# Yusin2Chen/incomplete_multimodal_fusion

Hardware: AMD Instinct MI355X
Metric: pretrain_samples_per_sec (higher is better)
Workload: dtype bf16

## Files before the change

incomplete_multimodal_fusion_amd/csrc/mha_sh.hip:

```cpp
#include "mha_common.hpp"
#include "mmae_hip.h"

typedef short s16x4 __attribute__((ext_vector_type(4)));
typedef short s16x8 __attribute__((ext_vector_type(8)));
typedef float f32x16 __attribute__((ext_vector_type(16)));
typedef unsigned u32x4 __attribute__((ext_vector_type(4)));
typedef unsigned u32x2 __attribute__((ext_vector_type(2)));
typedef __bf16 bf16x2 __attribute__((ext_vector_type(2)));
#define LDS_AS __attribute__((address_space(3)))

#ifndef SH_SKEW
#define SH_SKEW 0
#endif
#ifndef SH_SLEEP_CLASS
#define SH_SLEEP_CLASS (-1)
#endif
#define SH_NS 4
#define SH_D 3
#define SH_MAXT 64
#define SH_MAXP 64
#define SH_LOG2E 1.4426950408889634f
#define SH_LN2 0.6931471805599453f
#define SH_THR 6.0f

__device__ __forceinline__ int sh_uni(int v) { return __builtin_amdgcn_readfirstlane(v); }
__device__ __forceinline__ int sh_f(int r) { return (((r >> 1) & 1) << 2) | (((r >> 2) & 1) << 1) | ((r >> 3) & 1); }
__device__ __forceinline__ float sh_exp2(float x) { return __builtin_amdgcn_exp2f(x); }
__device__ __forceinline__ f32x16 sh_mma(const bf16x8& a, const bf16x8& b, const f32x16& c) {
    return __builtin_amdgcn_mfma_f32_32x32x16_bf16(a, b, c, 0, 0, 0);
}
__device__ __forceinline__ float sh_swap_max(float v) {
    const unsigned w = __builtin_bit_cast(unsigned, v);
    auto b = __builtin_amdgcn_permlane32_swap(w, w, false, false);
    return fmaxf(__builtin_bit_cast(float, (unsigned)b[0]), __builtin_bit_cast(float, (unsigned)b[1]));
}
__device__ __forceinline__ float sh_swap_sum(float v) {
    const unsigned w = __builtin_bit_cast(unsigned, v);
    auto b = __builtin_amdgcn_permlane32_swap(w, w, false, false);
    return __builtin_bit_cast(float, (unsigned)b[0]) + __builtin_bit_cast(float, (unsigned)b[1]);
}
#define SH_W1(k) "s_waitcnt vmcnt(" #k ")\n\ts_branch .Lshw_end_%=\n\t"
#define SH_W4(a, b, c, d) SH_W1(a) SH_W1(b) SH_W1(c) SH_W1(d)
__device__ __forceinline__ void sh_wait_vm(int n) {
    int k = sh_uni(n < 0 ? 0 : (n > 31 ? 31 : n));
    asm volatile(
        "s_getpc_b64 vcc\n\t"
        "s_lshl_b32 %0, %0, 3\n\t"
        "s_add_u32 %0, %0, 20\n\t"
        "s_add_u32 vcc_lo, vcc_lo, %0\n\t"
        "s_addc_u32 vcc_hi, vcc_hi, 0\n\t"
        "s_setpc_b64 vcc\n\t"
        SH_W4(0, 1, 2, 3) SH_W4(4, 5, 6, 7) SH_W4(8, 9, 10, 11) SH_W4(12, 13, 14, 15)
        SH_W4(16, 17, 18, 19) SH_W4(20, 21, 22, 23) SH_W4(24, 25, 26, 27) SH_W4(28, 29, 30, 31)
        ".Lshw_end_%=:"
        : "+s"(k) : : "vcc", "scc", "memory");
}
__device__ __forceinline__ float sh_bf16_round(float x) { return (float)(bf16)x; }
__device__ __forceinline__ unsigned sh_pack2(float lo, float hi) {
    const unsigned a = __builtin_bit_cast(unsigned short, (bf16)lo), b = __builtin_bit_cast(unsigned short, (bf16)hi);
    return a | (b << 16);
}
__device__ __forceinline__ bf16x8 sh_ext(unsigned w0) { return __builtin_bit_cast(bf16x8, u32x4{w0, 0u, 0u, 0u}); }

struct ShSeg {
    int qlen, qst, klen, kst;
    __device__ __forceinline__ void load(const MhaDesc& p, int b, int lane) {
        const int i = b * p.nseg + (lane < p.nseg ? lane : 0);
        qlen = p.q_len[i]; qst = p.q_start[i]; klen = p.k_len[i]; kst = p.k_start[i];
    }
    __device__ __forceinline__ int ql(int s) const { return __builtin_amdgcn_readlane(qlen, sh_uni(s)); }
    __device__ __forceinline__ int qs(int s) const { return __builtin_amdgcn_readlane(qst, sh_uni(s)); }
    __device__ __forceinline__ int kl(int s) const { return __builtin_amdgcn_readlane(klen, sh_uni(s)); }
    __device__ __forceinline__ int ks(int s) const { return __builtin_amdgcn_readlane(kst, sh_uni(s)); }
};

__device__ __forceinline__ void sh_dma(const bf16* base, int n_rows, int row_bytes, int voff, int soff, bf16* lds_piece) {
    const unsigned long long a = reinterpret_cast<unsigned long long>(base);
    const unsigned lo = __builtin_amdgcn_readfirstlane((unsigned)a), hi = __builtin_amdgcn_readfirstlane((unsigned)(a >> 32));
    bf16* ub = reinterpret_cast<bf16*>(((unsigned long long)hi << 32) | lo);
    const __amdgpu_buffer_rsrc_t rs = __builtin_amdgcn_make_buffer_rsrc(ub, 0, sh_uni(n_rows * row_bytes), 0x00020000);
    __builtin_amdgcn_raw_ptr_buffer_load_lds(rs, (LDS_AS void*)lds_piece, 16, voff, sh_uni(soff), 0, 0);
}

__device__ __forceinline__ void sh_dma4(const float* base, int n, float* lds, int lane) {
    const unsigned long long a = reinterpret_cast<unsigned long long>(base);
    const unsigned lo = __builtin_amdgcn_readfirstlane((unsigned)a), hi = __builtin_amdgcn_readfirstlane((unsigned)(a >> 32));
    float* ub = reinterpret_cast<float*>(((unsigned long long)hi << 32) | lo);
    const __amdgpu_buffer_rsrc_t rs = __builtin_amdgcn_make_buffer_rsrc(ub, 0, sh_uni(n * 4), 0x00020000);
    int z = 0;
    asm volatile("" : "+s"(z));
    __builtin_amdgcn_raw_ptr_buffer_load_lds(rs, (LDS_AS void*)lds, 4, (lane + z) * 4, 0, 0, 0);
}

__device__ __forceinline__ u32x4 sh_rsrc_words(const void* base, int bytes) {
    const unsigned long long a = reinterpret_cast<unsigned long long>(base);
    return u32x4{(unsigned)__builtin_amdgcn_readfirstlane((unsigned)a), (unsigned)__builtin_amdgcn_readfirstlane((unsigned)(a >> 32)) & 0xffffu,
                 (unsigned)sh_uni(bytes), 0x00020000u};
}
__device__ __forceinline__ u32x4 sh_ld128_async(const void* base, int bytes, int voff) {
    u32x4 v;
    asm volatile("s_nop 4\n\tbuffer_load_dwordx4 %0, %1, %2, 0 offen" : "=&v"(v) : "v"(voff), "s"(sh_rsrc_words(base, bytes)) : "memory");
    return v;
}
__device__ __forceinline__ unsigned sh_ld32_async(const void* base, int bytes, int voff) {
    unsigned v;
    asm volatile("s_nop 4\n\tbuffer_load_dword %0, %1, %2, 0 offen" : "=&v"(v) : "v"(voff), "s"(sh_rsrc_words(base, bytes)) : "memory");
    return v;
}
__device__ __forceinline__ void sh_pin(u32x4& a, u32x4& b, unsigned& c) { asm volatile("" : "+v"(a), "+v"(b), "+v"(c)); }
template <int CTRL>
__device__ __forceinline__ float sh_add_dpp(float x) {
    return x + __builtin_bit_cast(float, __builtin_amdgcn_update_dpp(0, __builtin_bit_cast(int, x), CTRL, 0xf, 0xf, true));
}

__device__ __forceinline__ bf16x8 sh_tr(const bf16* img, int off0, int off1) {
    const s16x4 lo = __builtin_amdgcn_ds_read_tr16_b64_v4i16((LDS_AS s16x4*)(img + off0));
    const s16x4 hi = __builtin_amdgcn_ds_read_tr16_b64_v4i16((LDS_AS s16x4*)(img + off1));
    s16x8 x;
    x[0] = lo[0]; x[1] = lo[1]; x[2] = lo[2]; x[3] = lo[3]; x[4] = hi[0]; x[5] = hi[1]; x[6] = hi[2]; x[7] = hi[3];
    return __builtin_bit_cast(bf16x8, x);
}
__device__ __forceinline__ bf16x8 sh_ld8(const bf16* p) { return *reinterpret_cast<const bf16x8*>(p); }

struct ShAddr {
    int krow0, tr00;
    __device__ __forceinline__ void init(int lane) {
        const int r = lane & 31, hh = lane >> 5;
        krow0 = r * 64 + 8 * (hh ^ sh_f(r));
        const int g16 = lane >> 4, q = (lane & 15) >> 2, pp = lane & 3;
        const int row = 4 * (g16 >> 1) + q, ch = 2 * (g16 & 1) + (pp >> 1);
        tr00 = row * 64 + 8 * (ch ^ sh_f(row)) + 4 * (pp & 1);
    }
};

struct ShSlot {
    bf16x8 q[4];
    f32x16 o[2];
    float mref, lsum;
    unsigned ext;
    int row;
    int nq;
};

#ifndef MMAE_DIAG
#define MMAE_DIAG 1
#endif
#define SH_STAMP_WAVES (MMAE_DIAG ? 8192 : 1)
__device__ unsigned long long g_sh_stamps[SH_STAMP_WAVES][16];
__device__ __forceinline__ unsigned long long sh_now() {
    unsigned long long t;
    asm volatile("s_memtime %0\n\ts_waitcnt lgkmcnt(0)" : "=s"(t) :: "memory");
    return t;
}
extern "C" int mmae_debug_sh_stamps(unsigned long long* host32) {
    if (!host32 || !MMAE_DIAG) return MMAE_ERR_ARG;
    static unsigned long long* h = nullptr;
    if (!h) h = new unsigned long long[(size_t)SH_STAMP_WAVES * 16];
    if (hipMemcpyFromSymbol(h, HIP_SYMBOL(g_sh_stamps), sizeof(unsigned long long) * SH_STAMP_WAVES * 16) != hipSuccess) return MMAE_ERR_LAUNCH;
    for (int i = 0; i < 32; ++i) host32[i] = 0;
    for (size_t w = 0; w < SH_STAMP_WAVES; ++w)
        for (int i = 0; i < 16; ++i) host32[16 * ((w & 15) >= 8) + i] += h[w * 16 + i];
    void* dptr = nullptr;
    if (hipGetSymbolAddress(&dptr, HIP_SYMBOL(g_sh_stamps)) != hipSuccess) return MMAE_ERR_LAUNCH;
    if (hipMemset(dptr, 0, sizeof(unsigned long long) * SH_STAMP_WAVES * 16) != hipSuccess) return MMAE_ERR_LAUNCH;
    return MMAE_OK;
}
#define SH_T(i) do { if (ST) { __builtin_amdgcn_sched_barrier(0); const unsigned long long n__ = sh_now(); tt[i] += n__ - tl; tl = n__; __builtin_amdgcn_sched_barrier(0); } } while (0)

template <bool ST>
__device__ __forceinline__ void sh_attend(ShSlot& s, bool fresh, const bf16* Kst, const bf16* Vst, int stage_el, const ShAddr& ad,
                                          const unsigned (&kext)[2], int hh, unsigned long long (&tt)[16], unsigned long long& tl) {
    f32x16 sacc[2];
    const bf16x8 qe = sh_ext(s.ext);
    const int kbase = ad.krow0 + stage_el, vbase = ad.tr00 + stage_el;
    f32x16 z;
#pragma unroll
    for (int i = 0; i < 16; ++i) z[i] = 0.f;
#pragma unroll
    for (int kb = 0; kb < 2; ++kb) {
        bf16x8 kf[4];
#pragma unroll
        for (int ks = 0; ks < 4; ++ks) kf[ks] = sh_ld8(Kst + 2048 * kb + (kbase ^ (16 * ks)));
        sacc[kb] = sh_mma(sh_ext(kext[kb]), qe, z);
#pragma unroll
        for (int ks = 0; ks < 4; ++ks) sacc[kb] = sh_mma(kf[ks], s.q[ks], sacc[kb]);
        __builtin_amdgcn_sched_group_barrier(0x100, 4, 0);
        __builtin_amdgcn_sched_group_barrier(0x008, 5, 0);
    }
    if (ST) asm volatile("s_nop 15\n\ts_nop 15\n\ts_nop 15\n\ts_nop 15" ::: "memory");
    SH_T(4);
    float mx0 = fmaxf(sacc[0][0], sacc[0][1]), mx1 = fmaxf(sacc[1][0], sacc[1][1]);
#pragma unroll
    for (int i = 2; i < 16; i += 2) { mx0 = fmaxf(fmaxf(mx0, sacc[0][i]), sacc[0][i + 1]); mx1 = fmaxf(fmaxf(mx1, sacc[1][i]), sacc[1][i + 1]); }
    const float mx = sh_swap_max(fmaxf(mx0, mx1));
    const bool need = fresh | (mx > SH_THR);
    if (__builtin_amdgcn_ballot_w64(need) != 0) {
        const float want = s.mref + (fresh ? mx : fmaxf(mx, 0.f));
        const float mnew = sh_bf16_round(want);
        const float delta = mnew - s.mref;
        if (!fresh) {
            const float alpha = sh_exp2(-delta);
            s.lsum *= alpha;
#pragma unroll
            for (int d = 0; d < 2; ++d)
#pragma unroll
                for (int i = 0; i < 16; ++i) s.o[d][i] *= alpha;
        }
        s.mref = mnew;
        s.ext = hh == 0 ? sh_pack2(-mnew, 1.0f) : 0u;
#pragma unroll
        for (int kb = 0; kb < 2; ++kb)
#pragma unroll
            for (int i = 0; i < 16; ++i) sacc[kb][i] -= delta;
    }
    bf16x8 pb[2][2];
    const bf16x2 ones = {(bf16)1.0f, (bf16)1.0f};
#pragma unroll
    for (int kb = 0; kb < 2; ++kb) {
#pragma unroll
        for (int i = 0; i < 16; ++i) sacc[kb][i] = sh_exp2(sacc[kb][i]);
#pragma unroll
        for (int s2 = 0; s2 < 2; ++s2) {
#pragma unroll
            for (int j = 0; j < 8; ++j) pb[kb][s2][j] = (bf16)sacc[kb][8 * s2 + j];
            const u32x4 w = __builtin_bit_cast(u32x4, pb[kb][s2]);
#pragma unroll
            for (int j = 0; j < 4; ++j) s.lsum = __builtin_amdgcn_fdot2_f32_bf16(__builtin_bit_cast(bf16x2, (unsigned)w[j]), ones, s.lsum, false);
        }
    }
    SH_T(5);
#pragma unroll
    for (int kb = 0; kb < 2; ++kb) {
#pragma unroll
        for (int s2 = 0; s2 < 2; ++s2) {
            const bf16* vb = Vst + 64 * (32 * kb + 16 * s2);
            if (kb == 0 && s2 == 0 && fresh) {
#pragma unroll
                for (int d = 0; d < 2; ++d) s.o[d] = sh_mma(sh_tr(vb, vbase ^ (32 * d), vbase ^ (32 * d + 520)), pb[kb][s2], z);
            } else {
#pragma unroll
                for (int d = 0; d < 2; ++d) s.o[d] = sh_mma(sh_tr(vb, vbase ^ (32 * d), vbase ^ (32 * d + 520)), pb[kb][s2], s.o[d]);
            }
        }
        if (kb == 0) __builtin_amdgcn_sched_barrier(0);
    }
    if (ST) asm volatile("s_nop 15\n\ts_nop 15\n\ts_nop 15\n\ts_nop 15" ::: "memory");
    SH_T(6);
}

__device__ __forceinline__ void sh_finish(const ShSlot& s, const MhaDesc& p, int h, int r, int hh) {
    const float lq = sh_swap_sum(s.lsum);
    const float inv = lq > 0.f ? 1.f / lq : 0.f;
    const bool valid = r < s.nq;
    bf16* op = reinterpret_cast<bf16*>(p.o) + (long)s.row * p.o_stride + h * 64 + 8 * hh;
#pragma unroll
    for (int d = 0; d < 2; ++d)
#pragma unroll
        for (int i = 0; i < 4; i += 2) {
            unsigned a0 = sh_pack2(s.o[d][4 * i] * inv, s.o[d][4 * i + 1] * inv), a1 = sh_pack2(s.o[d][4 * i + 2] * inv, s.o[d][4 * i + 3] * inv);
            unsigned b0 = sh_pack2(s.o[d][4 * i + 4] * inv, s.o[d][4 * i + 5] * inv), b1 = sh_pack2(s.o[d][4 * i + 6] * inv, s.o[d][4 * i + 7] * inv);
            auto r0 = __builtin_amdgcn_permlane32_swap(a0, b0, false, false); a0 = r0[0]; b0 = r0[1];
            auto r1 = __builtin_amdgcn_permlane32_swap(a1, b1, false, false); a1 = r1[0]; b1 = r1[1];
            if (valid) *reinterpret_cast<u32x4*>(op + 32 * d + 8 * i) = u32x4{a0, a1, b0, b1};
        }
    if (valid && hh == 0) p.lse[(long)h * p.stat_stride + s.row] = lq > 0.f ? s.mref * SH_LN2 + __logf(lq) : 0.f;
}

__device__ __forceinline__ void sh_zero_rows(const MhaDesc& p, long row0, int n, int h, int tid) {
    for (int i = tid; i < n * 8; i += 1024) {
        const int rr = i >> 3, c = i & 7;
        *reinterpret_cast<u32x4*>(reinterpret_cast<bf16*>(p.o) + (row0 + rr) * p.o_stride + h * 64 + 8 * c) = u32x4{0u, 0u, 0u, 0u};
        if (c == 0) p.lse[(long)h * p.stat_stride + row0 + rr] = 0.f;
    }
}

// ... 779 lines not shown
        for (int s = 0; s < fus; ++s) {
            const int nb = (st.kl(s) + 31) >> 5;
            if (nb == 0) continue;
            const int room = (SB_W - NB % SB_W) % SB_W;
            if (room > 0 && nb > room && nb <= SB_W) {
                const int pad = min(room, FB - fus_used);
                if (pad > 0) { place(fus, fus_used, pad); fus_used += pad; }
            }
            place(s, 0, nb);
        }
        if (FB > fus_used) place(fus, fus_used, FB - fus_used);
        NB = min(NB, SB_MAXB);
        npass = (NB + SB_W - 1) / SB_W;
        if (wave == 0) { kb_row_s[lane] = kb_row; kb_info_s[lane] = kb_info; }
        unsigned firstp = 0, lastp = 0, seen = 0;
        for (int ps = 0; ps < npass; ++ps)
            for (int w = 0; w < SB_W; ++w) {
                const int kbi = SB_W * ps + w;
                if (kbi < NB) {
                    const int s = (__builtin_amdgcn_readlane(kb_info, kbi) >> 8) & 15;
                    if (!((seen >> s) & 1)) { seen |= 1u << s; firstp |= (unsigned)ps << (4 * s); }
                    lastp = (lastp & ~(15u << (4 * s))) | ((unsigned)ps << (4 * s));
                }
            }
        for (int ps = 0; ps < npass; ++ps) {
            int segmask = 0;
            for (int w = 0; w < SB_W; ++w) {
                const int kbi = SB_W * ps + w;
                if (kbi < NB) segmask |= 1 << ((__builtin_amdgcn_readlane(kb_info, kbi) >> 8) & 15);
            }
            const int first = nsteps;
            int tbase = 0;
            for (int sq = 0; sq < nseg; ++sq) {
                const int QL = st.ql(sq), nt = (QL + 63) >> 6;
                const int tb = tbase;
                tbase += nt;
                if (QL == 0) continue;
                int mode = 0;
                if (sq == fus) mode = 1;
                else if (st.kl(sq) > 0) mode = (segmask >> sq) & 1;
                else if (p.empty_mode == 0) mode = 2;
                if (!mode) continue;
                const int fp = sq == fus ? 0 : (int)((firstp >> (4 * sq)) & 15), lp = sq == fus ? npass - 1 : (int)((lastp >> (4 * sq)) & 15);
#pragma unroll
                for (int k = 0; k < 2; ++k) {
                    const int j = lane + 64 * k - nsteps;
                    if (j >= 0 && j < nt) {
                        st_row[k] = st.qs(sq) + 64 * j; st_tid[k] = tb + j;
                        st_info[k] = min(64, QL - 64 * j) | (sq << 8) | (mode << 12) | (ps << 16) | ((ps == fp ? 1 : 0) << 25) | ((ps == lp ? 1 : 0) << 26);
                    }
                }
                nsteps += nt;
            }
            if (nsteps == first) {
#pragma unroll
                for (int k = 0; k < 2; ++k)
                    if (lane + 64 * k == nsteps) { st_row[k] = 0; st_tid[k] = 0; st_info[k] = (3 << 12) | (ps << 16); }
                ++nsteps;
            }
#pragma unroll
            for (int k = 0; k < 2; ++k)
                if (lane + 64 * k == nsteps - 1) st_info[k] |= 1 << 24;
        }
        nsteps = min(nsteps, SB_MAXS);
    }
    __syncthreads();
    for (int hi = 0; hi < hpb; ++hi)
        for (int s = 0; s < nseg; ++s) {
            const int QL = st.ql(s);
            if (QL > 0 && (NB == 0 || (s < fus && st.kl(s) == 0))) {
                const long row0 = st.qs(s);
                for (int i = tid; i < QL * 8; i += SB_W * 64)
                    *reinterpret_cast<u32x4*>(reinterpret_cast<bf16*>(p.dq) + (row0 + (i >> 3)) * p.dq_stride + (h0 + hi) * 64 + 8 * (i & 7)) = u32x4{0u, 0u, 0u, 0u};
            }
        }
    if (NB == 0) return;
    auto s_row = [&](int i) { return i < 64 ? __builtin_amdgcn_readlane(st_row[0], i) : __builtin_amdgcn_readlane(st_row[1], i - 64); };
    auto s_info = [&](int i) { return i < 64 ? __builtin_amdgcn_readlane(st_info[0], i) : __builtin_amdgcn_readlane(st_info[1], i - 64); };
    auto s_tid = [&](int i) { return i < 64 ? __builtin_amdgcn_readlane(st_tid[0], i) : __builtin_amdgcn_readlane(st_tid[1], i - 64); };

    const bf16* qg = reinterpret_cast<const bf16*>(p.q);
    const bf16* dog = reinterpret_cast<const bf16*>(p.dout);
    const bf16* kg = reinterpret_cast<const bf16*>(p.k);
    const bf16* vg = reinterpret_cast<const bf16*>(p.v);
    const int qsb = (int)p.q_stride * 2, dosb = (int)p.do_stride * 2, ksb = (int)p.k_stride * 2, vsb = (int)p.v_stride * 2;
    auto dma_voff = [&](int row_bytes, int z) { const int pr = (lane >> 3) + z; return pr * row_bytes + 16 * ((lane & 7) ^ sh_f(pr)); };
    ShAddr ad; ad.init(lane);
    const float cq = p.scale * SH_LOG2E;
    const int G = hpb * nsteps;
    int vm = 0, myseq = 0, mark = 0;
    int lj = 0, li = 0, lh = 0, lstage = 0;
    auto issue_ring = [&]() {
        if (wave == 4 + (lj & 3)) {
            const long row0 = s_row(li); const int n = s_info(li) & 255, h = h0 + lh;
            const bf16* qb_ = qg + row0 * p.q_stride + h * 64;
            const bf16* ob_ = dog + row0 * p.do_stride + h * 64;
            int z = 0;
            asm volatile("" : "+s"(z));
            const int qv = dma_voff(qsb, z), ov = dma_voff(dosb, z);
#pragma unroll
            for (int pc = 0; pc < 8; ++pc) {
                sh_dma(qb_, n, qsb, qv ^ (16 * (pc & 1)), 8 * pc * qsb, &ringQ[lstage][pc * 512]);
                sh_dma(ob_, n, dosb, ov ^ (16 * (pc & 1)), 8 * pc * dosb, &ringO[lstage][pc * 512]);
            }
            if (!RC) {
                const float* lp = p.delta + ((long)p.H + h) * p.stat_stride + row0;
                const float* dp = p.delta + (2L * p.H + h) * p.stat_stride + row0;
                sh_dma4(lp, n, &ringL[lstage][0], lane);
                sh_dma4(dp, n, &ringL[lstage][64], lane);
            }
            vm += RC ? 16 : 18; myseq = vm;
        }
        ++lj;
        if (++lstage == SB_NS) lstage = 0;
        if (++li == nsteps) { li = 0; ++lh; }
    };
    u32x4 rc_o[2] = {{0u, 0u, 0u, 0u}, {0u, 0u, 0u, 0u}}, rc_d[2] = {{0u, 0u, 0u, 0u}, {0u, 0u, 0u, 0u}};
    unsigned rc_l = 0u;
    int rcseq = 0;
    const bool rc_wave = RC && wave >= 4;
    const int rc_row = 16 * (wave & 3) + (lane >> 2), rc_c = lane & 3;
    auto rc_issue = [&](int i, int hx) {
        const long row0 = s_row(i); const int n = s_info(i) & 255, h = h0 + hx;
        const int osb = (int)p.o_stride * 2;
        const bf16* ob = reinterpret_cast<const bf16*>(p.o) + row0 * p.o_stride + h * 64;
        const bf16* db = dog + row0 * p.do_stride + h * 64;
        rc_o[0] = sh_ld128_async(ob, n * osb, rc_row * osb + 32 * rc_c);
        rc_o[1] = sh_ld128_async(ob, n * osb, rc_row * osb + 32 * rc_c + 16);
        rc_d[0] = sh_ld128_async(db, n * dosb, rc_row * dosb + 32 * rc_c);
        rc_d[1] = sh_ld128_async(db, n * dosb, rc_row * dosb + 32 * rc_c + 16);
        rc_l = sh_ld32_async(p.lse + (long)h * p.stat_stride + row0, n * 4, rc_row * 4);
        vm += 5; rcseq = vm;
    };
    auto rc_finish = [&](int to_stage) {
        sh_wait_vm(vm - rcseq);
        sh_pin(rc_o[0], rc_d[0], rc_l);
        sh_pin(rc_o[1], rc_d[1], rc_l);
        float acc = 0.f;
#pragma unroll
        for (int k = 0; k < 2; ++k) {
            const bf16x8 a = __builtin_bit_cast(bf16x8, rc_o[k]), d8 = __builtin_bit_cast(bf16x8, rc_d[k]);
#pragma unroll
            for (int j = 0; j < 8; ++j) acc += (float)a[j] * (float)d8[j];
        }
        acc = sh_add_dpp<0xB1>(acc);
        acc = sh_add_dpp<0x4E>(acc);
        if (rc_c == 0) {
            ringL[to_stage][rc_row] = -__builtin_bit_cast(float, rc_l) * SH_LOG2E;
            ringL[to_stage][64 + rc_row] = -acc;
        }
        asm volatile("s_waitcnt lgkmcnt(0)" ::: "memory");
    };
    auto kb_of = [&](int ps) { return SB_W * ps + wave; };
    bf16x8 vnext[4];
    auto issue_kv = [&](int ps, int h, int buf) {
        const int kbi = kb_of(ps);
        const long row0 = sh_uni(kb_row_s[kbi]); const int n = sh_uni(kb_info_s[kbi]) & 255;
        int z = 0;
        asm volatile("" : "+s"(z));
        const int kv_ = dma_voff(ksb, z);
#pragma unroll
        for (int j = 0; j < 4; ++j) sh_dma(kg + row0 * p.k_stride + h * 64, n, ksb, kv_ ^ (16 * (j & 1)), 8 * j * ksb, &kimg[buf][wave][8 * j * 64]);
        const bf16* vb = vg + row0 * p.v_stride + h * 64;
        const unsigned long long a = reinterpret_cast<unsigned long long>(vb);
        const unsigned lo = __builtin_amdgcn_readfirstlane((unsigned)a), hi = __builtin_amdgcn_readfirstlane((unsigned)(a >> 32));
        bf16* ub = reinterpret_cast<bf16*>(((unsigned long long)hi << 32) | lo);
        const __amdgpu_buffer_rsrc_t rs = __builtin_amdgcn_make_buffer_rsrc(ub, 0, sh_uni(n * vsb), 0x00020000);
#pragma unroll
        for (int ks = 0; ks < 4; ++ks)
            vnext[ks] = __builtin_bit_cast(bf16x8, __builtin_amdgcn_raw_buffer_load_b128(rs, (r + z) * vsb + 32 * ks + 16 * hh, 0, 0));
        vm += 8;
    };

    bf16x8 kf[4], vf[4];
    f32x16 dk[2], dv[2];
    int my_seg = -1, my_row = 0, my_n = 0;
    bool have = false;
    int nvalid = 0;
    const int dq_d = wave & 1, dq_q = (wave >> 1) & 1;
    const int dsw = (32 * wave + r) * 64, dsf = sh_f(r);

    int nxt_ps = 0, nxt_h = 0, cur_buf = 0, nxt_buf = 0;
    bool nxt_valid = kb_of(0) < NB;
    int rci = 0, rch = 0;
    auto rc_issue_next = [&]() { rc_issue(rci, rch); if (++rci == nsteps) { rci = 0; ++rch; } };
    if (rc_wave) rc_issue_next();
    if (nxt_valid) issue_kv(0, h0, 0);
    mark = vm;
    for (int i = 0; i < SB_D && i < G; ++i) issue_ring();
    if (rc_wave) { rc_finish(0); if (G > 1) rc_issue_next(); }

    int si = 0, hi = 0, stage = 0, cur_ps = -1;
    for (int g = 0; g < G; ++g) {
        if (wave == 4 + (g & 3)) sh_wait_vm(vm - myseq);
        __builtin_amdgcn_s_barrier();
        if (lj < G) issue_ring();
        const int inf = s_info(si), qn = inf & 255, sq = (inf >> 8) & 15, mode = (inf >> 12) & 15, ps = (inf >> 16) & 255;
        const bool last = (inf >> 24) & 1, tfirst = (inf >> 25) & 1, tlast = (inf >> 26) & 1;
        const int h = h0 + hi;
        if (ps != cur_ps) {
            cur_ps = ps;
            cur_buf = nxt_buf;
            have = kb_of(ps) < NB;
            if (have) {
                int z = 0;
                asm volatile("" : "+s"(z));
                const int kbi = kb_of(ps);
                const int ki = sh_uni(kb_info_s[kbi]);
                my_row = sh_uni(kb_row_s[kbi]); my_n = ki & 255; my_seg = (ki >> 8) & 15;
                sh_wait_vm(vm - mark);
                const int kbase = ad.krow0 + z;
#pragma unroll
                for (int ks = 0; ks < 4; ++ks) {
                    const bf16x8 raw = sh_ld8(&kimg[cur_buf][wave][0] + (kbase ^ (16 * ks)));
#pragma unroll
                    for (int j = 0; j < 8; ++j) kf[ks][j] = (bf16)((float)raw[j] * cq);
                    vf[ks] = vnext[ks];
                }
#pragma unroll
                for (int d = 0; d < 2; ++d)
#pragma unroll
                    for (int i = 0; i < 16; ++i) { dk[d][i] = 0.f; dv[d][i] = 0.f; }
            }
            nvalid = min(SB_W, NB - SB_W * ps);
            __builtin_amdgcn_sched_barrier(0);
            nxt_ps = ps + 1; nxt_h = hi;
            if (nxt_ps == npass) { nxt_ps = 0; ++nxt_h; }
            nxt_valid = nxt_h < hpb && kb_of(nxt_ps) < NB;
            nxt_buf = cur_buf ^ 1;
            if (nxt_valid) { issue_kv(nxt_ps, h0 + nxt_h, nxt_buf); mark = vm; }
        }
        const bool dq_wave = wave < 4 && mode == 1 && MODE != 1 && MODE != 4;
        f32x16 dqa;
        float* wsq = p.dq_ws + ((((long)b * p.max_qt + s_tid(si)) * p.H + h) * 4 + (2 * dq_d + dq_q)) * 1024 + 4 * lane;
        if (dq_wave && !tfirst && MODE == 0) {
#pragma unroll
            for (int i = 0; i < 4; ++i) {
                const f32x4 v4 = *reinterpret_cast<const f32x4*>(wsq + 256 * i);
                dqa[4 * i] = v4[0]; dqa[4 * i + 1] = v4[1]; dqa[4 * i + 2] = v4[2]; dqa[4 * i + 3] = v4[3];
            }
            vm += 4;
        } else {
#pragma unroll
            for (int i = 0; i < 16; ++i) dqa[i] = 0.f;
        }
        const bool part = have && (mode == 2 || (mode == 1 && (sq == fus || sq == my_seg)));
        if (MODE != 1 && mode == 1 && have && !part) {
#pragma unroll
            for (int c = 0; c < 8; ++c) *reinterpret_cast<u32x2*>(dsx + dsw + 8 * (c ^ dsf) + 4 * hh) = u32x2{0u, 0u};
        }
        if (part) {
            const bf16* Qs = ringQ[0]; const bf16* Os = ringO[0];
            const int sel = stage * 4096;
            const int rbase = ad.krow0 + sel, tbase = ad.tr00 + sel;
            const float* Ls = &ringL[stage][0];
#pragma unroll
            for (int qb = 0; qb < 2; ++qb) {
                bf16x8 pb[2], dsb[2];
                {
                    f32x16 sacc;
#pragma unroll
                    for (int j = 0; j < 4; ++j) {
                        const f32x4 a = *reinterpret_cast<const f32x4*>(Ls + 32 * qb + 8 * j + 4 * hh);
#pragma unroll
                        for (int i = 0; i < 4; ++i) sacc[4 * j + i] = a[i];
                    }
                    if (mode == 1)
#pragma unroll
                        for (int ks = 0; ks < 4; ++ks) sacc = sh_mma(sh_ld8(Qs + 2048 * qb + (rbase ^ (16 * ks))), kf[ks], sacc);
#pragma unroll
                    for (int s2 = 0; s2 < 2; ++s2)
#pragma unroll
                        for (int j = 0; j < 8; ++j) pb[s2][j] = (bf16)sh_exp2(sacc[8 * s2 + j]);
                }
                if (mode == 1) {
                    f32x16 dpacc;
#pragma unroll
                    for (int j = 0; j < 4; ++j) {
                        const f32x4 c = *reinterpret_cast<const f32x4*>(Ls + 64 + 32 * qb + 8 * j + 4 * hh);
#pragma unroll
                        for (int i = 0; i < 4; ++i) dpacc[4 * j + i] = c[i];
                    }
#pragma unroll
                    for (int ks = 0; ks < 4; ++ks) dpacc = sh_mma(sh_ld8(Os + 2048 * qb + (rbase ^ (16 * ks))), vf[ks], dpacc);
#pragma unroll
                    for (int s2 = 0; s2 < 2; ++s2) {
#pragma unroll
                        for (int j = 0; j < 8; ++j) dsb[s2][j] = (bf16)((float)pb[s2][j] * dpacc[8 * s2 + j]);
                        if (MODE != 1) {
                            const u32x4 w4 = __builtin_bit_cast(u32x4, dsb[s2]);
                            const int c0 = 4 * qb + 2 * s2;
                            *reinterpret_cast<u32x2*>(dsx + dsw + 8 * (c0 ^ dsf) + 4 * hh) = u32x2{w4[0], w4[1]};
                            *reinterpret_cast<u32x2*>(dsx + dsw + 8 * ((c0 + 1) ^ dsf) + 4 * hh) = u32x2{w4[2], w4[3]};
                        }
                    }
                } else {
#pragma unroll
                    for (int s2 = 0; s2 < 2; ++s2) dsb[s2] = __builtin_bit_cast(bf16x8, u32x4{0u, 0u, 0u, 0u});
                }
#pragma unroll
                for (int s2 = 0; s2 < 2; ++s2) {
                    const int ro = 64 * (32 * qb + 16 * s2);
#pragma unroll
                    for (int d = 0; d < 2; ++d) {
                        dv[d] = sh_mma(sh_tr(Os + ro, tbase ^ (32 * d), tbase ^ (32 * d + 520)), pb[s2], dv[d]);
                        dk[d] = sh_mma(sh_tr(Qs + ro, tbase ^ (32 * d), tbase ^ (32 * d + 520)), dsb[s2], dk[d]);
                    }
                    __builtin_amdgcn_sched_barrier(0);
                }
            }
        }
        if (last && have) {
            const bool valid = r < my_n;
            bf16* dkp = reinterpret_cast<bf16*>(p.dk) + (long)(my_row + r) * p.dk_stride + h * 64 + 8 * hh;
            bf16* dvp = reinterpret_cast<bf16*>(p.dv) + (long)(my_row + r) * p.dv_stride + h * 64 + 8 * hh;
#pragma unroll
            for (int d = 0; d < 2; ++d)
#pragma unroll
                for (int i = 0; i < 4; i += 2) {
                    unsigned a0 = sh_pack2(dk[d][4 * i] * p.scale, dk[d][4 * i + 1] * p.scale), a1 = sh_pack2(dk[d][4 * i + 2] * p.scale, dk[d][4 * i + 3] * p.scale);
                    unsigned b0 = sh_pack2(dk[d][4 * i + 4] * p.scale, dk[d][4 * i + 5] * p.scale), b1 = sh_pack2(dk[d][4 * i + 6] * p.scale, dk[d][4 * i + 7] * p.scale);
                    auto r0 = __builtin_amdgcn_permlane32_swap(a0, b0, false, false); a0 = r0[0]; b0 = r0[1];
                    auto r1 = __builtin_amdgcn_permlane32_swap(a1, b1, false, false); a1 = r1[0]; b1 = r1[1];
                    if (valid) *reinterpret_cast<u32x4*>(dkp + 32 * d + 8 * i) = u32x4{a0, a1, b0, b1};
                    unsigned c0 = sh_pack2(dv[d][4 * i], dv[d][4 * i + 1]), c1 = sh_pack2(dv[d][4 * i + 2], dv[d][4 * i + 3]);
                    unsigned e0 = sh_pack2(dv[d][4 * i + 4], dv[d][4 * i + 5]), e1 = sh_pack2(dv[d][4 * i + 6], dv[d][4 * i + 7]);
                    auto r2 = __builtin_amdgcn_permlane32_swap(c0, e0, false, false); c0 = r2[0]; e0 = r2[1];
                    auto r3 = __builtin_amdgcn_permlane32_swap(c1, e1, false, false); c1 = r3[0]; e1 = r3[1];
                    if (valid) *reinterpret_cast<u32x4*>(dvp + 32 * d + 8 * i) = u32x4{c0, c1, e0, e1};
                }
            vm += 8;
        }
        if (MODE != 1) {
            asm volatile("s_waitcnt lgkmcnt(0)" ::: "memory");
            __builtin_amdgcn_s_barrier();
        }
        if (rc_wave && g + 1 < G) {
            rc_finish(stage + 1 == SB_NS ? 0 : stage + 1);
            if (g + 2 < G) rc_issue_next();
        }
        if (dq_wave) {
            const bf16* Kc = &kimg[cur_buf][0][0];
            const int ka = ad.tr00 ^ (32 * dq_d), kb2 = ad.tr00 ^ (32 * dq_d + 520), sa = ad.tr00 ^ (32 * dq_q), sb2 = ad.tr00 ^ (32 * dq_q + 520);
            if (nvalid == SB_W) {
#pragma unroll
                for (int w = 0; w < SB_W; ++w)
#pragma unroll
                    for (int ks = 0; ks < 2; ++ks) {
                        const int ro = 64 * (32 * w + 16 * ks);
                        dqa = sh_mma(sh_tr(Kc + ro, ka, kb2), sh_tr(dsx + ro, sa, sb2), dqa);
                    }
            } else {
                for (int w = 0; w < nvalid; ++w)
#pragma unroll
                    for (int ks = 0; ks < 2; ++ks) {
                        const int ro = 64 * (32 * w + 16 * ks);
                        dqa = sh_mma(sh_tr(Kc + ro, ka, kb2), sh_tr(dsx + ro, sa, sb2), dqa);
                    }
            }
            if (!tlast && MODE == 2) {
                asm volatile("" :: "v"(dqa));
            } else if (!tlast) {
#pragma unroll
                for (int i = 0; i < 4; ++i)
                    *reinterpret_cast<f32x4*>(wsq + 256 * i) = f32x4{dqa[4 * i], dqa[4 * i + 1], dqa[4 * i + 2], dqa[4 * i + 3]};
                vm += 4;
            } else {
                const int qr = 32 * dq_q + r;
                const bool valid = qr < qn;
                bf16* dqp = reinterpret_cast<bf16*>(p.dq) + (long)(s_row(si) + qr) * p.dq_stride + h * 64 + 32 * dq_d + 8 * hh;
                if (qn > 32 * dq_q) {
#pragma unroll
                    for (int i = 0; i < 4; i += 2) {
                        unsigned a0 = sh_pack2(dqa[4 * i] * p.scale, dqa[4 * i + 1] * p.scale), a1 = sh_pack2(dqa[4 * i + 2] * p.scale, dqa[4 * i + 3] * p.scale);
                        unsigned b0 = sh_pack2(dqa[4 * i + 4] * p.scale, dqa[4 * i + 5] * p.scale), b1 = sh_pack2(dqa[4 * i + 6] * p.scale, dqa[4 * i + 7] * p.scale);
                        auto r0 = __builtin_amdgcn_permlane32_swap(a0, b0, false, false); a0 = r0[0]; b0 = r0[1];
                        auto r1 = __builtin_amdgcn_permlane32_swap(a1, b1, false, false); a1 = r1[0]; b1 = r1[1];
                        if (valid) *reinterpret_cast<u32x4*>(dqp + 8 * i) = u32x4{a0, a1, b0, b1};
                    }
                    vm += 2;
                }
            }
        }
        if (++stage == SB_NS) stage = 0;
        if (++si == nsteps) { si = 0; ++hi; cur_ps = -1; }
    }
}

static int sh_heads_per_block(int B, int H, int req) {
    if (req > 0 && req <= H && H % req == 0) return req;
    int hpb = H;
    while (hpb > 1 && (long)B * (H / hpb) < 256) {
        int d = hpb - 1;
        while (d > 1 && H % d) --d;
        hpb = d;
    }
    return hpb;
}

bool mha_sh_applicable(const MhaDesc& d) {
    return d.max_q_rows >= 128 && d.max_k_rows / 64 + d.nseg <= SH_MAXT && d.k_stride == d.v_stride && d.nseg <= MAXSEG &&
           d.max_q_rows / 256 + 2 * d.nseg <= SH_MAXP;
}

int mha_sh_fwd(const MhaDesc& d, int mode, hipStream_t st) {
    if (d.max_k_rows / 64 + d.nseg > SH_MAXT || d.k_stride != d.v_stride || d.nseg > MAXSEG) return MMAE_ERR_ARG;
    const int hpb = sh_heads_per_block(d.B, d.H, d.hpb_req);
    const dim3 grid(d.B * (d.H / hpb)), blk(1024);
    if (mode == 1) MMAE_LAUNCH((mha_sh_fwd_kernel<1, 0>), grid, blk, 0, st, d, hpb);
    else if (mode == 2) MMAE_LAUNCH((mha_sh_fwd_kernel<2, 0>), grid, blk, 0, st, d, hpb);
#if MMAE_DIAG
    else if (mode == 3) MMAE_LAUNCH((mha_sh_fwd_kernel<3, 0>), grid, blk, 0, st, d, hpb);
#else
    else if (mode == 3) return MMAE_ERR_ARG;
#endif
    else if (mode == 10) MMAE_LAUNCH((mha_sh_fwd_kernel<0, 1>), grid, blk, 0, st, d, hpb);
    else if (mode == 11) MMAE_LAUNCH((mha_sh_fwd_kernel<1, 1>), grid, blk, 0, st, d, hpb);
    else if (mode == 12) MMAE_LAUNCH((mha_sh_fwd_kernel<2, 1>), grid, blk, 0, st, d, hpb);
    else if (mode == 4) MMAE_LAUNCH((mha_sh_fwd_kernel<4, 0>), grid, blk, 0, st, d, hpb);
    else if (mode == 20) MMAE_LAUNCH((mha_sh_fwd_kernel<0, 2>), grid, blk, 0, st, d, hpb);
    else if (mode == 21) MMAE_LAUNCH((mha_sh_fwd_kernel<1, 2>), grid, blk, 0, st, d, hpb);
    else MMAE_LAUNCH((mha_sh_fwd_kernel<0, 0>), grid, blk, 0, st, d, hpb);
    MMAE_CHECK_LAUNCH();
    return MMAE_OK;
}

bool mha_sh_dkdv_supported(const MhaDesc& d) {
    const int nb = d.max_k_rows / 32 + d.nseg, passes = (nb + SD_W - 1) / SD_W;
    return nb <= SD_MAXB && d.nseg <= MAXSEG && passes * (d.max_q_rows / 64 + d.nseg + 1) <= SD_MAXS;
}

int mha_sh_dkdv(const MhaDesc& d, int mode, hipStream_t st) {
    if (!mha_sh_dkdv_supported(d)) return MMAE_ERR_ARG;
    const int hpb = sh_heads_per_block(d.B, d.H, d.hpb_req);
    const dim3 grid(d.B * (d.H / hpb)), blk(SD_W * 64);
    if (mode == 1) MMAE_LAUNCH(mha_sh_dkdv_kernel<1>, grid, blk, 0, st, d, hpb);
    else if (mode == 2) MMAE_LAUNCH(mha_sh_dkdv_kernel<2>, grid, blk, 0, st, d, hpb);
    else MMAE_LAUNCH(mha_sh_dkdv_kernel<0>, grid, blk, 0, st, d, hpb);
    MMAE_CHECK_LAUNCH();
    return MMAE_OK;
}

bool mha_sh_fused_supported(const MhaDesc& d) {
    const int nb = d.max_k_rows / 32 + d.nseg, passes = (nb + SB_W - 1) / SB_W;
    return nb <= SB_MAXB && passes <= 15 && d.nseg <= MAXSEG && d.H <= 8 && passes * (d.max_q_rows / 64 + d.nseg + 1) <= SB_MAXS && d.dq_ws != nullptr &&
           d.max_qt >= d.max_q_rows / 64 + d.nseg;
}

int mha_sh_bwd_fused(const MhaDesc& d, int mode, hipStream_t st) {
    if (!mha_sh_fused_supported(d)) return MMAE_ERR_ARG;
    if (mode != 3 && mode != 5) {
        MMAE_LAUNCH(mha_rowconst_kernel, dim3((unsigned)((d.stat_stride + 31) / 32)), dim3(256), 0, st, d);
        MMAE_CHECK_LAUNCH();
    }
    const int hpb = sh_heads_per_block(d.B, d.H, d.hpb_req);
    const dim3 grid(d.B * (d.H / hpb)), blk(SB_W * 64);
    if (mode == 1) MMAE_LAUNCH((mha_sh_bwd_kernel<1, false>), grid, blk, 0, st, d, hpb);
    else if (mode == 2) MMAE_LAUNCH((mha_sh_bwd_kernel<2, false>), grid, blk, 0, st, d, hpb);
    else if (mode == 4) MMAE_LAUNCH((mha_sh_bwd_kernel<4, false>), grid, blk, 0, st, d, hpb);
    else if (mode == 5) MMAE_LAUNCH((mha_sh_bwd_kernel<0, true>), grid, blk, 0, st, d, hpb);
    else MMAE_LAUNCH((mha_sh_bwd_kernel<0, false>), grid, blk, 0, st, d, hpb);
    MMAE_CHECK_LAUNCH();
    return MMAE_OK;
}

bool mha_sh_dq_supported(const MhaDesc& d) {
    return d.max_k_rows / 64 + d.nseg <= SQ_MAXT && d.nseg <= MAXSEG && d.max_q_rows / 128 + 1 <= SQ_MAXP;
}

int mha_sh_dq(const MhaDesc& d, int mode, hipStream_t st) {
    if (!mha_sh_dq_supported(d)) return MMAE_ERR_ARG;
    const int hpb = sh_heads_per_block(d.B, d.H, d.hpb_req);
    const dim3 grid(d.B * (d.H / hpb)), blk(SQ_W * 64);
    if (mode == 1) MMAE_LAUNCH(mha_sh_dq_kernel<1>, grid, blk, 0, st, d, hpb);
    else if (mode == 2) MMAE_LAUNCH(mha_sh_dq_kernel<2>, grid, blk, 0, st, d, hpb);
    else MMAE_LAUNCH(mha_sh_dq_kernel<0>, grid, blk, 0, st, d, hpb);
    MMAE_CHECK_LAUNCH();
    return MMAE_OK;
}
```

Measured before the change: 1626.

## Use async inline-asm loads for V and dQ workspace, swizzle dS stores

Replaces the compiler-generated buffer loads for V tiles and for the dQ workspace accumulator with inline-asm async buffer loads that are waited on explicitly, just before use, using vm counters. The dQ load is issued early and consumed only in the dq phase, so its latency can overlap the dS computation. The dS LDS stores now go through explicit ds_write_b64 with an extra half-swizzle on the lane's row parity, and the transposed read addresses are adjusted to match, to reduce bank conflicts. This carries correctness risk in the vm-count bookkeeping and in keeping the store and read swizzles consistent.

```diff
diff --git a/incomplete_multimodal_fusion_amd/csrc/mha_sh.hip b/incomplete_multimodal_fusion_amd/csrc/mha_sh.hip
--- a/incomplete_multimodal_fusion_amd/csrc/mha_sh.hip
+++ b/incomplete_multimodal_fusion_amd/csrc/mha_sh.hip
@@ -108,6 +108,7 @@
     return v;
 }
 __device__ __forceinline__ void sh_pin(u32x4& a, u32x4& b, unsigned& c) { asm volatile("" : "+v"(a), "+v"(b), "+v"(c)); }
+__device__ __forceinline__ void sh_pin(u32x4& a, u32x4& b) { asm volatile("" : "+v"(a), "+v"(b)); }
 template <int CTRL>
 __device__ __forceinline__ float sh_add_dpp(float x) {
     return x + __builtin_bit_cast(float, __builtin_amdgcn_update_dpp(0, __builtin_bit_cast(int, x), CTRL, 0xf, 0xf, true));
@@ -121,6 +122,10 @@
     return __builtin_bit_cast(bf16x8, x);
 }
 __device__ __forceinline__ bf16x8 sh_ld8(const bf16* p) { return *reinterpret_cast<const bf16x8*>(p); }
+__device__ __forceinline__ void sh_st64(bf16* p, u32x2 v) {
+    const unsigned a = (unsigned)(__UINTPTR_TYPE__)(LDS_AS bf16*)p;
+    asm volatile("ds_write_b64 %0, %1" :: "v"(a), "v"(v) : "memory");
+}
 
 struct ShAddr {
     int krow0, tr00;
@@ -1206,7 +1211,7 @@
         asm volatile("s_waitcnt lgkmcnt(0)" ::: "memory");
     };
     auto kb_of = [&](int ps) { return SB_W * ps + wave; };
-    bf16x8 vnext[4];
+    u32x4 vnext[4];
     auto issue_kv = [&](int ps, int h, int buf) {
         const int kbi = kb_of(ps);
         const long row0 = sh_uni(kb_row_s[kbi]); const int n = sh_uni(kb_info_s[kbi]) & 255;
@@ -1216,13 +1221,8 @@
 #pragma unroll
         for (int j = 0; j < 4; ++j) sh_dma(kg + row0 * p.k_stride + h * 64, n, ksb, kv_ ^ (16 * (j & 1)), 8 * j * ksb, &kimg[buf][wave][8 * j * 64]);
         const bf16* vb = vg + row0 * p.v_stride + h * 64;
-        const unsigned long long a = reinterpret_cast<unsigned long long>(vb);
-        const unsigned lo = __builtin_amdgcn_readfirstlane((unsigned)a), hi = __builtin_amdgcn_readfirstlane((unsigned)(a >> 32));
-        bf16* ub = reinterpret_cast<bf16*>(((unsigned long long)hi << 32) | lo);
-        const __amdgpu_buffer_rsrc_t rs = __builtin_amdgcn_make_buffer_rsrc(ub, 0, sh_uni(n * vsb), 0x00020000);
-#pragma unroll
-        for (int ks = 0; ks < 4; ++ks)
-            vnext[ks] = __builtin_bit_cast(bf16x8, __builtin_amdgcn_raw_buffer_load_b128(rs, (r + z) * vsb + 32 * ks + 16 * hh, 0, 0));
+#pragma unroll
+        for (int ks = 0; ks < 4; ++ks) vnext[ks] = sh_ld128_async(vb, n * vsb, (r + z) * vsb + 32 * ks + 16 * hh);
         vm += 8;
     };
 
@@ -1232,7 +1232,7 @@
     bool have = false;
     int nvalid = 0;
     const int dq_d = wave & 1, dq_q = (wave >> 1) & 1;
-    const int dsw = (32 * wave + r) * 64, dsf = sh_f(r);
+    const int dsw = (32 * wave + r) * 64, dsf = sh_f(r), dsh = 4 * (hh ^ (r & 1));
 
     int nxt_ps = 0, nxt_h = 0, cur_buf = 0, nxt_buf = 0;
     bool nxt_valid = kb_of(0) < NB;
@@ -1263,13 +1263,15 @@
                 const int ki = sh_uni(kb_info_s[kbi]);
                 my_row = sh_uni(kb_row_s[kbi]); my_n = ki & 255; my_seg = (ki >> 8) & 15;
                 sh_wait_vm(vm - mark);
+                sh_pin(vnext[0], vnext[1]);
+                sh_pin(vnext[2], vnext[3]);
                 const int kbase = ad.krow0 + z;
 #pragma unroll
                 for (int ks = 0; ks < 4; ++ks) {
                     const bf16x8 raw = sh_ld8(&kimg[cur_buf][wave][0] + (kbase ^ (16 * ks)));
 #pragma unroll
                     for (int j = 0; j < 8; ++j) kf[ks][j] = (bf16)((float)raw[j] * cq);
-                    vf[ks] = vnext[ks];
+                    vf[ks] = __builtin_bit_cast(bf16x8, vnext[ks]);
                 }
 #pragma unroll
                 for (int d = 0; d < 2; ++d)
@@ -1285,23 +1287,20 @@
             if (nxt_valid) { issue_kv(nxt_ps, h0 + nxt_h, nxt_buf); mark = vm; }
         }
         const bool dq_wave = wave < 4 && mode == 1 && MODE != 1 && MODE != 4;
-        f32x16 dqa;
-        float* wsq = p.dq_ws + ((((long)b * p.max_qt + s_tid(si)) * p.H + h) * 4 + (2 * dq_d + dq_q)) * 1024 + 4 * lane;
-        if (dq_wave && !tfirst && MODE == 0) {
-#pragma unroll
-            for (int i = 0; i < 4; ++i) {
-                const f32x4 v4 = *reinterpret_cast<const f32x4*>(wsq + 256 * i);
-                dqa[4 * i] = v4[0]; dqa[4 * i + 1] = v4[1]; dqa[4 * i + 2] = v4[2]; dqa[4 * i + 3] = v4[3];
-            }
-            vm += 4;
-        } else {
-#pragma unroll
-            for (int i = 0; i < 16; ++i) dqa[i] = 0.f;
+        const float* wsq0 = p.dq_ws + ((((long)b * p.max_qt + s_tid(si)) * p.H + h) * 4 + (2 * dq_d + dq_q)) * 1024;
+        float* wsq = const_cast<float*>(wsq0) + 4 * lane;
+        const bool dq_ld = dq_wave && !tfirst && MODE == 0;
+        u32x4 dqw[4];
+        int dqseq = 0;
+        if (dq_ld) {
+#pragma unroll
+            for (int i = 0; i < 4; ++i) dqw[i] = sh_ld128_async(wsq0, 4096, 16 * lane + 1024 * i);
+            vm += 4; dqseq = vm;
         }
         const bool part = have && (mode == 2 || (mode == 1 && (sq == fus || sq == my_seg)));
         if (MODE != 1 && mode == 1 && have && !part) {
 #pragma unroll
-            for (int c = 0; c < 8; ++c) *reinterpret_cast<u32x2*>(dsx + dsw + 8 * (c ^ dsf) + 4 * hh) = u32x2{0u, 0u};
+            for (int c = 0; c < 8; ++c) sh_st64(dsx + dsw + 8 * (c ^ dsf) + dsh, u32x2{0u, 0u});
         }
         if (part) {
             const bf16* Qs = ringQ[0]; const bf16* Os = ringO[0];
@@ -1344,8 +1343,8 @@
                         if (MODE != 1) {
                             const u32x4 w4 = __builtin_bit_cast(u32x4, dsb[s2]);
                             const int c0 = 4 * qb + 2 * s2;
-                            *reinterpret_cast<u32x2*>(dsx + dsw + 8 * (c0 ^ dsf) + 4 * hh) = u32x2{w4[0], w4[1]};
-                            *reinterpret_cast<u32x2*>(dsx + dsw + 8 * ((c0 + 1) ^ dsf) + 4 * hh) = u32x2{w4[2], w4[3]};
+                            sh_st64(dsx + dsw + 8 * (c0 ^ dsf) + dsh, u32x2{w4[0], w4[1]});
+                            sh_st64(dsx + dsw + 8 * ((c0 + 1) ^ dsf) + dsh, u32x2{w4[2], w4[3]});
                         }
                     }
                 } else {
@@ -1394,8 +1393,23 @@
             if (g + 2 < G) rc_issue_next();
         }
         if (dq_wave) {
+            f32x16 dqa;
+            if (dq_ld) {
+                sh_wait_vm(vm - dqseq);
+                sh_pin(dqw[0], dqw[1]);
+                sh_pin(dqw[2], dqw[3]);
+#pragma unroll
+                for (int i = 0; i < 4; ++i) {
+                    const f32x4 v4 = __builtin_bit_cast(f32x4, dqw[i]);
+                    dqa[4 * i] = v4[0]; dqa[4 * i + 1] = v4[1]; dqa[4 * i + 2] = v4[2]; dqa[4 * i + 3] = v4[3];
+                }
+            } else {
+#pragma unroll
+                for (int i = 0; i < 16; ++i) dqa[i] = 0.f;
+            }
             const bf16* Kc = &kimg[cur_buf][0][0];
-            const int ka = ad.tr00 ^ (32 * dq_d), kb2 = ad.tr00 ^ (32 * dq_d + 520), sa = ad.tr00 ^ (32 * dq_q), sb2 = ad.tr00 ^ (32 * dq_q + 520);
+            const int trd = ad.tr00 ^ (4 * ((lane >> 2) & 1));
+            const int ka = ad.tr00 ^ (32 * dq_d), kb2 = ad.tr00 ^ (32 * dq_d + 520), sa = trd ^ (32 * dq_q), sb2 = trd ^ (32 * dq_q + 520);
             if (nvalid == SB_W) {
 #pragma unroll
                 for (int w = 0; w < SB_W; ++w)
```

After: 1627 (median of 6 runs). No clear change (+0.0%).
